# MiroBeno/Volume-Rendering

Hardware: AMD Instinct MI355X
Metric: Mrays/s (W*H / t_frame), 1024^3 volume @ 2048^2 viewport (higher is better)
Workload: dtype f32

## Files before the change

### include/vr_hip.h

```cpp
#ifndef VR_HIP_H
#define VR_HIP_H

#include <stddef.h>
#include <stdint.h>

#ifdef __cplusplus
extern "C" {
#endif

#define VR_TF_SIZE          128
#define VR_TF_RATIO         2
#define VR_ESL_VOLUME_DIMS  32
#define VR_ESL_VOLUME_SIZE  1024
#define VR_ESL_MIN_BLOCK    8

typedef enum vr_status {
	VR_OK               = 0,
	VR_ERR_INVALID      = 1,
	VR_ERR_NO_DEVICE    = 2,
	VR_ERR_ALLOC        = 3,
	VR_ERR_HIP          = 4,
	VR_ERR_NOT_READY    = 5
} vr_status;

// ... 72 lines not shown
int vr_hip_render_device(vr_ctx *ctx, const vr_params *params, void *dev_rgba, void *stream);

int vr_hip_render_mip(vr_ctx *ctx, const vr_params *params, uint8_t *host_rgba);
int vr_hip_render_mip_device(vr_ctx *ctx, const vr_params *params, void *dev_rgba, void *stream);

typedef struct vr_launch_info {
	uint32_t layout;
	uint32_t brick_plane;
	uint32_t lane_map;
	uint32_t phase_x, phase_y;
	uint32_t clamp_fetch;
	uint32_t tiles_x, tiles_y;
	uint32_t ordered;
	uint32_t straddle_permille;
	uint32_t column_voxels;
} vr_launch_info;
int vr_hip_last_launch(vr_ctx *ctx, vr_launch_info *out);

int vr_hip_timing(vr_ctx *ctx, vr_timing *out);
int vr_hip_timing_reset(vr_ctx *ctx);

int vr_hip_volume_minmax(vr_ctx *ctx, uint8_t *minmax_out, uint32_t *esl_block_dims_out, float *esl_block_size_out,
                         float *kernel_ms_out);
int vr_hip_volume_histogram(vr_ctx *ctx, uint64_t *hist256_out, float *kernel_ms_out);

int vr_hip_generate_volume(vr_ctx *ctx, uint32_t kind, uint32_t n, uint32_t seed, uint32_t bytes_per_voxel);
int vr_hip_download_volume(vr_ctx *ctx, void *host_out, uint64_t bytes);

typedef struct vr_multi vr_multi;
int  vr_hip_multi_create(int n, const int *devices, vr_multi **out);
// ... 62 lines not shown
```

### volume-rendering_amd/binding.py

```python
import ctypes as C
import os

SAMPLE_NEAREST = 0
SAMPLE_TRILINEAR = 1
SAMPLE_TRILINEAR_Q8 = 2
LAYOUT_LINEAR = 0
LAYOUT_BRICKED = 1
COPY_QUAD_XY, COPY_QUAD_XZ, COPY_QUAD_YZ, COPY_RUN_Z, COPY_RUN_Y, COPY_VOXEL, COPY_OCT, COPY_COL_X, COPY_COL_Y, COPY_COL_Z, COPY_ALL = 1, 2, 4, 8, 16, 32, 64, 128, 256, 512, 8191
COPY_COLV_X, COPY_COLV_Y, COPY_COLV_Z = 1024, 2048, 4096
COPY_NAMES = ("quad_xy", "quad_xz", "quad_yz", "run_z", "run_y", "voxel", "oct", "col_x", "col_y", "col_z", "colv_x", "colv_y", "colv_z")
COPY_KINDS = 13
TF_SIZE = 128
ESL_VOLUME_SIZE = 1024

_STATUS = {0: "VR_OK", 1: "VR_ERR_INVALID", 2: "VR_ERR_NO_DEVICE", 3: "VR_ERR_ALLOC", 4: "VR_ERR_HIP", 5: "VR_ERR_NOT_READY"}


class VrError(RuntimeError):
    def __init__(self, code, message=""):
        self.code = code
        super().__init__(f"{_STATUS.get(code, code)}: {message}" if message else _STATUS.get(code, str(code)))


class VrView(C.Structure):
# ... 22 lines not shown
class VrVolumeInfo(C.Structure):
    _fields_ = [("dim_x", C.c_uint32), ("dim_y", C.c_uint32), ("dim_z", C.c_uint32), ("bytes_per_voxel", C.c_uint32),
                ("layout", C.c_uint32), ("brick_copies", C.c_uint32), ("brick_copies_wanted", C.c_uint32), ("brick_planes", C.c_uint32),
                ("linear_resident", C.c_uint32), ("run_copy", C.c_uint32), ("linear_bytes", C.c_uint64), ("bricked_bytes", C.c_uint64),
                ("copies", C.c_uint32), ("copies_in_policy", C.c_uint32), ("copies_refused", C.c_uint32),
                ("build_ms", C.c_float * 13), ("upload_ms", C.c_float)]


class VrTiming(C.Structure):
    _fields_ = [("kernel_ms", C.c_float), ("total_ms", C.c_float), ("launches", C.c_uint64), ("kernel_ms_sum", C.c_double),
                ("kernel_ms_max", C.c_float), ("total_ms_max", C.c_float)]


class VrLaunchInfo(C.Structure):
    _fields_ = [(n, C.c_uint32) for n in ("layout", "brick_plane", "lane_map", "phase_x", "phase_y", "clamp_fetch", "tiles_x", "tiles_y",
                                          "ordered", "straddle_permille", "column_voxels")]


def library_path():
    return os.environ.get("VR_HIP_LIB") or os.path.join(os.path.dirname(os.path.abspath(__file__)), "libvr_hip.so")


_lib = None


def lib():
    global _lib
    if _lib is not None:
        return _lib
    import torch
    path = library_path()
# ... 84 lines not shown
```

### volume-rendering_amd/csrc/vr_device.h

```cpp
#pragma once

#include <hip/hip_runtime.h>
#include <stdint.h>
#include "../../include/vr_hip.h"

namespace vr {

constexpr uint32_t kMaxRaySteps = 1u << 22;

#ifndef VR_DEPTH
#define VR_DEPTH 5
#endif
constexpr int kDepth = VR_DEPTH, kSlots = kDepth + 1;
#ifndef VR_LAZY_EXIT
#define VR_LAZY_EXIT 1
#endif
#ifndef VR_RUN_DEPTH
#define VR_RUN_DEPTH VR_DEPTH
#endif
constexpr int kDepthTwoByte = 3;
constexpr int kRunDepth = VR_RUN_DEPTH, kMaxDepth = kRunDepth > kDepth ? kRunDepth : kDepth;
constexpr int kOverrunSteps = kMaxDepth + (VR_LAZY_EXIT ? kMaxDepth + 1 : 0);
constexpr int kLutPad = (kOverrunSteps * 5 + 2) / 3 + 2;
static_assert(kDepth >= 1 && kDepth <= 6 && kRunDepth >= 1 && kRunDepth <= 12, "prefetch depth");
// ... 26 lines not shown
	uint32_t dual_shift;
	uint32_t dual_bits[32];
	uint32_t col_axis;
	struct ColDenseSample {
		float ax, ay, az;
		float tf_scale;
		float max_x, max_y, max_z;
		float tf_zero_below;
		float light_kd, ray_threshold;
		uint32_t pad[2];
	} col_sample;
	struct ColDenseShade {
		float dir[3];  float kd_scaled;
		float light[3]; uint32_t nbu;
		float lh[3];   uint32_t nw;
		uint32_t dim[3], pad;
	} col_shade;
#ifdef VR_BOUNDS_CHECK
	uint64_t bc_base, bc_bytes;
	uint64_t bc_alt_bytes;
	uint32_t *bc_fault;
	uint32_t bc_ntiles;
#endif
};
#ifndef VR_TILE_ORDER
#define VR_TILE_ORDER 8
#endif
#ifndef VR_XCD_MODE
#define VR_XCD_MODE 5
#endif
inline void tile_number_to_xy(uint32_t tile, uint32_t tiles_x, uint32_t tiles_y, uint32_t *x, uint32_t *y) {
// ... 119 lines not shown
```

### volume-rendering_amd/csrc/vr_hip_api.cpp

```cpp
#include "vr_device.h"

#include <algorithm>
#include <chrono>
#include <cmath>
#include <cstdio>
#include <cstdlib>
#include <cstring>
#include <new>
#include <string>
#include <vector>

using namespace vr;

#ifndef VR_ORDER_ALWAYS
#define VR_ORDER_ALWAYS 0
#endif

namespace {

constexpr int kEventRing = 256;

struct EventPair { hipEvent_t start = nullptr, stop = nullptr; bool pending = false; };

}
// ... 349 lines not shown
}

#ifdef VR_BOUNDS_CHECK
hipError_t bounds_check_arm(vr_ctx *c, RayKernelArgs &a, const vr_params *p, const RaymarchPlan &plan, const void *brick_copy, uint32_t ntiles) {
	if (c->bc_fault == nullptr) {
		hipError_t e = hipMalloc((void **) &c->bc_fault, 8 * sizeof(uint32_t));
		if (e == hipSuccess) e = hipMemset(c->bc_fault, 0, 8 * sizeof(uint32_t));
		if (e != hipSuccess) return e;
	}
	const void *array = plan.reads_linear ? c->vol : brick_copy;
	const bool column = a.layout == kLayoutColumn || a.layout == kLayoutVoxCol;
	a.bc_base = (uint64_t) (uintptr_t) array - (column ? kColPadBytes : 0u);
	a.bc_bytes = plan.reads_linear ? (c->vol_elems + volume_tail_slack(c->dim[0], c->dim[1])) * c->bpv :
	             copy_bytes(c, copy_kind_of(a, p->sampling));
	if (column) a.bc_bytes += 2ull * kColPadBytes;
	a.bc_alt_bytes = a.alt_copy ? copy_bytes(c, kCopyRunY) : 0;
	a.bc_fault = c->bc_fault; a.bc_ntiles = ntiles;
	if (const char *e = getenv("VR_BC_SELFTEST")) if (atoi(e) == 1) a.bc_bytes /= 2;
	return hipSuccess;
}

int bounds_check_verdict(vr_ctx *c, hipStream_t stream, uint32_t layout) {
	uint32_t fault[6] = { 0, 0, 0, 0, 0, 0 };
	VR_TRY(c, hipStreamSynchronize(stream));
	VR_TRY(c, hipMemcpy(fault, c->bc_fault, sizeof fault, hipMemcpyDeviceToHost));
	if (fault[0] != 0u) {
		char msg[256];
		snprintf(msg, sizeof msg, "bounds check: code %u (1 table index [axis << 8], 2 offset, 3 address, 4 cost slot) workgroup %u thread %u value 0x%08x%08x limit %u, layout %u",
		         fault[0], fault[1], fault[2], fault[4], fault[3], fault[5], layout);
		(void) hipMemset(c->bc_fault, 0, 8 * sizeof(uint32_t));
		return fail(c, VR_ERR_HIP, msg);
// ... 90 lines not shown
		if (hit == nullptr) {
			const uint32_t straddle = choose_tile_mapping(a);
			hit = &c->map_cache[c->map_next];
			hit->straddle_permille = straddle;
			if (hit->dual_state != 0 || hit->order_tiles != 0) VR_TRY(c, drain(c));
			hit->dual_state = 0; hit->order_tiles = 0;
			constexpr uint32_t kMaps = sizeof c->map_cache / sizeof c->map_cache[0];
			c->map_next = (c->map_next + 1) % kMaps;
			if (c->map_cached < kMaps) c->map_cached++;
			hit->p = *p; memcpy(hit->dim, c->dim, sizeof c->dim);
			hit->lane_map = a.lane_map; hit->phase_x = a.phase_x; hit->phase_y = a.phase_y;
		}
		a.lane_map = hit->lane_map; a.phase_x = hit->phase_x; a.phase_y = hit->phase_y;
		if (run_if_unaligned && hit->straddle_permille > 150u && copy_possible(c, run_layout == kLayoutRunY ? kCopyRunY : kCopyRunZ)) a.layout = run_layout;
	}
	bool dual_analytic = false;
	int dual_stage = -1;
	const bool dual_test = c->brick_plane_force == (int) kPlanes + 4, dual_measured = c->brick_plane_force == (int) kPlanes + 3;
	if (dual_candidate && is_run_layout(a.layout) && !p->esl && p->ray_threshold >= 1.0f && !a.clamp_fetch && c->bpv == 1 &&
	    copy_possible(c, kCopyRunZ) && copy_possible(c, kCopyRunY)) {
		if (dual_test || dual_measured) {
			if (hit != nullptr && c->tile_scheduling == 1 && !VR_ORDER_ALWAYS) {
				dual_stage = dual_test ? 4 : (int) hit->dual_state;
				a.layout = dual_stage == 4 ? kLayoutRunDual : ((dual_stage & 1) ? kLayoutRunY : kLayoutRun);
			}
		} else {
			dual_analytic = true;
			a.layout = kLayoutRunDual;
		}
	}
	static const bool col_ert = [] { const char *e = getenv("VR_COL_ERT"); return e == nullptr || atoi(e) != 0; }();
	if (bricked && c->bpv == 1 && !c->force_wide && !p->view.perspective && !p->esl && (p->ray_threshold >= 1.0f || col_ert) &&
	    !a.clamp_fetch && c->column_force >= 0 && (c->brick_plane_force < 0 || c->column_force > 0)) {
		const float *d = va.d;
		const int m = va.major;
		const float advance = d[m] * p->ray_step;
		bool take = advance >= 1.0f / 64.0f && advance <= 1.0f && one_cell_per_pixel(p, half);
		if (c->column_force == 0)
			for (int i = 0; i < 3; i++) if (i != m && d[i] * 4.0f >= 0.45f) take = false;
		const bool nearest = p->sampling == VR_SAMPLE_NEAREST;
		bool voxcol = false;
		if (!nearest && c->column_copy == 0 && col_copy_bytes(c->dim, (uint32_t) m, true) < (1ull << 32)) {
			auto span = [&](int i) { return (int) std::floor(7.0f * (std::fabs(p->view.right_plane[i]) + std::fabs(p->view.up_plane[i])) * half[i]) + 4; };
			voxcol = span(m == 0 ? 1 : 0) * span(m == 2 ? 1 : 2) <= 64;
		}
		if (take && copy_possible(c, (nearest || voxcol ? kCopyColVoxX : kCopyColX) + (uint32_t) m)) {
			a.layout = voxcol ? kLayoutVoxCol : kLayoutColumn; a.col_axis = (uint32_t) m; a.brick_plane = (uint32_t) m;
			a.col_sample.ax = p->view.direction[0] * a.half_x; a.col_sample.ay = p->view.direction[1] * a.half_y; a.col_sample.az = p->view.direction[2] * a.half_z;
			a.col_sample.tf_scale = a.tf_scale; a.col_sample.tf_zero_below = a.tf_zero_below;
			a.col_sample.max_x = a.max_x; a.col_sample.max_y = a.max_y; a.col_sample.max_z = a.max_z;
			a.col_sample.light_kd = p->light_kd; a.col_sample.ray_threshold = p->ray_threshold;
			for (int i = 0; i < 3; i++) { a.col_shade.dir[i] = p->view.direction[i]; a.col_shade.light[i] = p->view.light_pos[i]; }
			a.col_shade.lh[0] = a.lh_x; a.col_shade.lh[1] = a.lh_y; a.col_shade.lh[2] = a.lh_z;
			a.col_shade.kd_scaled = a.kd_scaled;
			for (int i = 0; i < 3; i++) a.col_shade.dim[i] = c->dim[i];
			a.col_shade.nbu = col_blocks(c->dim[m == 0 ? 1 : 0]);
			a.col_shade.nw = col_windows(c->dim[m], nearest || voxcol ? kColVoxCells : kColCells);
			dual_analytic = false; dual_stage = -1;
		}
	}
	const void *brick_copy = nullptr;
	if (a.layout == kLayoutRunDual) {
		brick_copy = copy_for(c, kCopyRunZ);
		a.alt_copy = (uint64_t) (uintptr_t) copy_for(c, kCopyRunY);
		if (brick_copy == nullptr || a.alt_copy == 0) { a.layout = run_layout; dual_stage = -1; dual_analytic = false; brick_copy = nullptr; }
	}
	if (a.layout != kLayoutLinear && brick_copy == nullptr) {
		const uint32_t want = copy_kind_of(a, p->sampling);
		brick_copy = copy_for(c, want);
		if (brick_copy == nullptr && want != kCopyQuadXY) {
			a.layout = kLayoutBricked; a.brick_plane = kPlaneXY;
			forget_tile_mappings(c);
			brick_copy = copy_for(c, kCopyQuadXY);
		}
		if (brick_copy == nullptr) brick_copy = resident_fallback(c, p->sampling, true, a.layout);
	}
	if (c->tile_lane_map < 0 && is_run_layout(a.layout) && p->view.perspective && !p->esl) {
		if (va.along) {
			const int run_axis = a.layout == kLayoutRunY ? 1 : 2;
			const float across = std::fabs(p->view.right_plane[run_axis]), down = std::fabs(p->view.up_plane[run_axis]);
			a.lane_map = (a.lane_map & 3u) | ((down > across ? 2u : 1u) << 2);
		}
	}
	if (c->tile_lane_map < 0 && a.layout == kLayoutVoxel && p->view.perspective && (a.lane_map & 3u) == kLaneBlocks) {
		if (va.major != 2) a.lane_map = std::fabs(p->view.up_plane[2]) > std::fabs(p->view.right_plane[2]) ? kLaneColumns : kLaneRows;
	}
	const RaymarchPlan plan = plan_raymarch(a, brick_copy != nullptr, c->bpv);
	if (plan.reads_linear && c->vol == nullptr)
		return fail(c, VR_ERR_NOT_READY, "this frame needs the linear array, which was released (vr_hip_release_linear_copy): no resident brick copy "
		                                 "serves this sampling mode / addressing path — prepare it before releasing, or set the volume again");

// ... 110 lines not shown
	if (c->tile_scheduling == 2 && ntiles <= (1u << 20)) {
		if (c->cost_map_capacity < ntiles) {
			VR_TRY(c, drain(c));
			if (c->cost_map) (void) hipFree(c->cost_map);
			c->cost_map = nullptr; c->cost_map_capacity = 0;
			VR_TRY(c, hipMalloc((void **) &c->cost_map, (size_t) ntiles * 4));
			c->cost_map_capacity = ntiles;
		}
		VR_TRY(c, hipMemsetAsync(c->cost_map, 0, (size_t) ntiles * 4, stream));
		sched.cost = c->cost_map;
		c->cost_map_tiles_x = plan.tiles_x; c->cost_map_tiles_y = plan.tiles_y;
	}

	c->last_launch = vr_launch_info{ a.layout == kLayoutVoxCol ? (uint32_t) kLayoutColumn : a.layout, a.brick_plane, a.lane_map, a.phase_x, a.phase_y, a.clamp_fetch,
	                                 plan.tiles_x, plan.tiles_y, sched.order != nullptr ? 1u : 0u, hit != nullptr ? hit->straddle_permille : 1000u,
	                                 a.layout == kLayoutVoxCol ? 1u : 0u };

	uint64_t frame_seq = 0;
	const int rc = launch_timed(c, a, p, plan, brick_copy, stream, frame_seq, [&] { return launch_raymarch(a, c->vol, brick_copy, c->bpv, c->tf, c->esl, dev_rgba, sched, stream); });
	if (rc) return rc;
	if (dual_advance) {
		if (dual_stage == 3) VR_TRY(c, launch_tile_choice(hit->cost, hit->order + hit->capacity, hit->order, ntiles, stream));
		VR_TRY(c, hipEventRecord(hit->order_ready, stream));
		hit->order_stream = stream; hit->order_tiles = ntiles;
		hit->dual_state = (uint32_t) dual_stage + 1u;
	}
	if (read_slot != nullptr) read_slot->last_seq = frame_seq;
	if (record_slot != nullptr) {
		VR_TRY(c, launch_tile_order(record_slot->cost, record_slot->order, ntiles, stream));
		VR_TRY(c, hipEventRecord(record_slot->ready, stream));
		record_slot->valid = true; record_slot->ntiles = ntiles; record_slot->stream = stream; record_slot->issue_seq = record_slot->last_seq = frame_seq;
// ... 165 lines not shown
		if (hit == nullptr) {
			constexpr uint32_t kMaps = sizeof c->mip_map / sizeof c->mip_map[0];
			hit = &c->mip_map[c->mip_map_next];
			c->mip_map_next = (c->mip_map_next + 1) % kMaps;
			if (c->mip_mapped < kMaps) c->mip_mapped++;
			hit->straddle_permille = choose_tile_mapping(a);
			hit->p = *p; memcpy(hit->dim, c->dim, sizeof c->dim); hit->layout = a.layout; hit->brick_plane = a.brick_plane;
			hit->lane_map = a.lane_map; hit->phase_x = a.phase_x; hit->phase_y = a.phase_y;
		}
		a.lane_map = hit->lane_map; a.phase_x = hit->phase_x; a.phase_y = hit->phase_y; straddle = hit->straddle_permille;
	}
	const RaymarchPlan plan = plan_raymarch(a, brick_copy != nullptr, c->bpv);
	if (plan.reads_linear && c->vol == nullptr)
		return fail(c, VR_ERR_NOT_READY, "this MIP frame needs the linear array, which was released (vr_hip_release_linear_copy): no resident brick copy "
		                                 "serves this sampling mode / addressing path — prepare it before releasing, or set the volume again");
	c->last_launch = vr_launch_info{ plan.reads_linear ? (uint32_t) kLayoutLinear : a.layout, a.brick_plane, a.lane_map, a.phase_x, a.phase_y, 0u, plan.tiles_x, plan.tiles_y, 0u, straddle, 0u };
	uint64_t frame_seq = 0;
	return launch_timed(c, a, p, plan, brick_copy, stream, frame_seq, [&] { return launch_mip(a, c->vol, brick_copy, c->bpv, c->tf, a.p.esl ? c->mip_bounds : nullptr, dev_rgba, stream); });
}

int render_preamble(vr_ctx *c, const vr_params *p, const void *buffer, bool host_frame) {
	if (c == nullptr) return VR_ERR_INVALID;
	if (buffer == nullptr) return fail(c, VR_ERR_INVALID, "buffer is NULL");
	int rc = validate_params(c, p);
	if (rc) return rc;
	rc = ready(c);
	if (rc) return rc;
	if (host_frame && (c->fb == nullptr || (size_t) p->out_width * p->out_rows * 4 > c->fb_bytes))
		return fail(c, VR_ERR_NOT_READY, "output larger than the window buffer: call vr_hip_set_window first");
	VR_TRY(c, hipSetDevice(c->device));
	return VR_OK;
// ... 166 lines not shown
		return VR_OK;
	}
	c->column_force = 0;
	if (plane < -1 || plane > (int32_t) kPlanes + 4)
		return fail(c, VR_ERR_INVALID, "plane must be -1 (per view), 0 (x,y), 1 (x,z), 2 (y,z), 3 (run bricks along z), 4 (run bricks along y), 5 (oct bricks for every view of a "
		                               "2-byte volume), 6 (both run copies, chosen per tile by measurement, for every full-march view), 7 (both run copies on alternating tiles), "
		                               "8 (column windows for every orthogonal full-march frame) or 9 (never the column windows)");
	c->oct_always = plane == (int32_t) kPlanes + 2;
	c->brick_plane_force = c->oct_always ? -1 : plane;
	forget_tile_mappings(c);
	return VR_OK;
}

int vr_hip_set_column_copy(vr_ctx *c, uint32_t mode) {
	if (c == nullptr) return VR_ERR_INVALID;
	if (mode > 1u) return fail(c, VR_ERR_INVALID, "column copy must be 0 (voxel windows where a wave's columns fit, else quad-element windows) or 1 (quad-element windows)");
	c->column_copy = mode;
	return VR_OK;
}

int vr_hip_set_tile_scheduling(vr_ctx *c, uint32_t mode) {
	if (c == nullptr) return VR_ERR_INVALID;
	if (mode > 2u) return fail(c, VR_ERR_INVALID, "tile scheduling mode must be 0 (workgroup id), 1 (measured-cost order) or 2 (workgroup id + cost map)");
	c->tile_scheduling = mode;
	forget_recorded_orders(c);
	return VR_OK;
}

int vr_hip_last_launch(vr_ctx *c, vr_launch_info *out) {
	if (c == nullptr || out == nullptr) return VR_ERR_INVALID;
	*out = c->last_launch;
// ... 264 lines not shown
```

### volume-rendering_amd/csrc/vr_kernels.hip

```cpp
#include "vr_device.h"
#include <initializer_list>

namespace vr {

#define VR_FMA(a, b, c) __builtin_fmaf((a), (b), (c))

struct f3 { float x, y, z; };
struct f4 { float x, y, z, w; };

__device__ __forceinline__ f3 mk3(float x, float y, float z) { f3 r; r.x = x; r.y = y; r.z = z; return r; }
__device__ __forceinline__ f3 ld3(const float *p) { return mk3(p[0], p[1], p[2]); }
__device__ __forceinline__ float flmin(float a, float b) { return a < b ? a : b; }
__device__ __forceinline__ float flmax(float a, float b) { return a > b ? a : b; }

__device__ __forceinline__ uint32_t map_float_int(float f, uint32_t n) {
	int i = (int) (f * (float) n);
	if (i >= (int) n) i = (int) n - 1;
	if (i < 0) i = 0;
	return (uint32_t) i;
}

struct __attribute__((aligned(16))) LdsTables {
	f4 tf[VR_TF_SIZE + 1];
	f4 dtf[VR_TF_SIZE + 1];
// ... 997 lines not shown
	w.flips_u = __builtin_amdgcn_ballot_w64(w.cu0 != w.cu1); w.flips_v = __builtin_amdgcn_ballot_w64(w.cv0 != w.cv1);
	w.ok = w.ok && __builtin_amdgcn_ballot_w64((w.cu1 - w.cu0) * (w.cu1 - w.cu0) > 1 || (w.cv1 - w.cv0) * (w.cv1 - w.cv0) > 1) == 0ull;
}
__device__ __forceinline__ bool col_lane_offsets(const ColWave &w, uint64_t stride_u, uint64_t stride_v, int64_t &ref, int64_t &rel0) {
	ref = (int64_t) col_lateral_offset64((uint32_t) __builtin_amdgcn_readlane(w.cu0, w.leader), (uint32_t) __builtin_amdgcn_readlane(w.cv0, w.leader), stride_u, stride_v);
	rel0 = (int64_t) col_lateral_offset64((uint32_t) w.cu0, (uint32_t) w.cv0, stride_u, stride_v) - ref;
	const int64_t du64 = (int64_t) col_axis_offset64((uint32_t) w.cu1, stride_u, kColWindowBytes) - (int64_t) col_axis_offset64((uint32_t) w.cu0, stride_u, kColWindowBytes);
	const int64_t dv64 = (int64_t) col_axis_offset64((uint32_t) w.cv1, stride_v, kColRowBytes) - (int64_t) col_axis_offset64((uint32_t) w.cv0, stride_v, kColRowBytes);
	const int64_t lim = 1ll << 28;
	return __builtin_amdgcn_ballot_w64(rel0 <= -lim || rel0 >= lim || du64 <= -lim || du64 >= lim || dv64 <= -lim || dv64 >= lim) == 0ull;
}
__device__ __forceinline__ uint64_t col_scalar_base(const uint8_t *copy, int64_t ref) {
	const uint64_t b = (uint64_t) (uintptr_t) copy + (uint64_t) ref - (1ull << 30);
	return ((uint64_t) rfl((uint32_t) (b >> 32)) << 32) | rfl((uint32_t) b);
}

struct ColBatch {
	float kvec, knext;
	int wvec;
	template <class W> __device__ __forceinline__ void refill(float step, uint32_t lane_i, W cell_to_window) {
		const float kbase = knext;
		const float k1 = kbase + step, delta = k1 - kbase, low = step - delta;
		const uint32_t e = __float_as_uint(kbase) >> 23;
		const float half_ulp = __uint_as_float((e > 24u ? e - 24u : 1u) << 23);
		const float kend = VR_FMA(64.0f, delta, kbase);
		const bool fast = rfl((e > 24u && (__float_as_uint(kend) >> 23) == e && __builtin_fabsf(low) != half_ulp && delta > 0.0f) ? 1u : 0u) != 0u;
		if (fast) {
			kvec = VR_FMA((float) lane_i, delta, kbase);
			knext = uni(kend);
		} else {
// ... 105 lines not shown
#if defined(VR_BOUNDS_CHECK)
		managed_load128(dst, VR_BC_ADDRESS(a, s_base + lane_offset, 16u));
#else
		managed_load128_s(dst, lane_offset, s_base);
#endif
		woff += dsign * (int) kColBlockBytes;
	}
	__device__ __forceinline__ bool careful(const ColEvents &e) {
		if (!FLIPS) return false;
		const int key = issue_key - (DEPTH + 1);
		while (key > cons_event) { cons_at++; cons_event = __builtin_amdgcn_readlane(e.events, cons_at & 63); }
		return key == cons_event;
	}
};

template <int SAMPLING, int M, class ShadeCorners>
__device__ __forceinline__ void col_tri_sample(const RayKernelArgs &a, uint32_t w0, uint32_t w1, float k, const f3 &B, ColRay &ray, uint64_t &live, f4 &acc,
                                               const f4 (&tf_l)[VR_TF_SIZE + 1], const f4 (&dtf_l)[VR_TF_SIZE + 1], const f4 (&org_l)[512], ShadeCorners shade_corners) {
	constexpr bool kQ8 = SAMPLING == VR_SAMPLE_TRILINEAR_Q8;
	if ((__builtin_amdgcn_uicmp((w0 | w1) & a.skip_mask, a.skip_cmp, kIcmpNE) & live) != 0ull && VR_OPEN_LANES(acc.w, live) != 0ull) {
		ColConstArgs q = col_dense_args();
		RayKernelArgs::ColDenseSample ds;
		ds.ax = q->col_sample.ax; ds.ay = q->col_sample.ay; ds.az = q->col_sample.az; ds.tf_scale = q->col_sample.tf_scale;
		ds.max_x = q->col_sample.max_x; ds.max_y = q->col_sample.max_y; ds.max_z = q->col_sample.max_z; ds.tf_zero_below = q->col_sample.tf_zero_below;
		ds.light_kd = q->col_sample.light_kd; ds.ray_threshold = q->col_sample.ray_threshold;
		hold_scalars(ds.ax, ds.ay, ds.az, ds.tf_scale, ds.max_x, ds.max_y, ds.max_z, ds.tf_zero_below, ds.light_kd, ds.ray_threshold);
		live &= __builtin_amdgcn_fcmpf(k, ray.ky, kFcmpOLE);
		const float xb = VR_FMA(k, ds.ax, B.x), yb = VR_FMA(k, ds.ay, B.y), zb = VR_FMA(k, ds.az, B.z);
		const float raw = col_resolve<M, kQ8>(w0, w1, ds.max_x, ds.max_y, ds.max_z, xb, yb, zb);
		const float tb = __builtin_amdgcn_fmed3f(VR_FMA(raw, ds.tf_scale, -0.5f), 0.0f, (float) (VR_TF_SIZE - 1));
		if ((__builtin_amdgcn_fcmpf(tb, ds.tf_zero_below, kFcmpOGE) & live) != 0ull) {
			f4 c;
			{
				const uint32_t i = (uint32_t) (int) tb;
				const float w = filter_weight<kQ8>(__builtin_amdgcn_fractf(tb));
				const f4 c0 = tf_l[i], dc = dtf_l[i];
				c.x = VR_FMA(w, dc.x, c0.x); c.y = VR_FMA(w, dc.y, c0.y); c.z = VR_FMA(w, dc.z, c0.z); c.w = VR_FMA(w, dc.w, c0.w);
			}
			const uint64_t shaded = ds.light_kd > 0.01f ? (__builtin_amdgcn_fcmpf(c.w, 0.05f, kFcmpOGT) & live) : 0ull;
			if (shaded != 0ull) {
				const f3 org = col_origin_again(org_l, ray.org_slot);
				RayKernelArgs::ColDenseShade dh;
				for (int i = 0; i < 3; i++) { dh.dir[i] = q->col_shade.dir[i]; dh.light[i] = q->col_shade.light[i]; dh.lh[i] = q->col_shade.lh[i]; }
				dh.kd_scaled = q->col_shade.kd_scaled; dh.nbu = q->col_shade.nbu; dh.nw = q->col_shade.nw;
				const uint8_t *const copy_p = ((ColConstKernelArguments) q)->copy;
				hold_scalars(dh.dir[0], dh.dir[1], dh.dir[2], dh.kd_scaled, dh.light[0], dh.light[1], dh.light[2], dh.lh[0], dh.lh[1], dh.lh[2]);
				hold_scalars(dh.nbu, dh.nw, (uint64_t) (uintptr_t) copy_p);
				const f3 p3 = march_point<SAMPLING>(org, mk3(dh.dir[0], dh.dir[1], dh.dir[2]), k);
				const f3 d = mk3(dh.light[0] - p3.x, dh.light[1] - p3.y, dh.light[2] - p3.z);
				const float inv = rsqrt_nr(VR_FMA(d.z, d.z, VR_FMA(d.y, d.y, d.x * d.x)));
				const float sx = VR_FMA(d.x * inv, dh.lh[0], xb), sy = VR_FMA(d.y * inv, dh.lh[1], yb), sz = VR_FMA(d.z * inv, dh.lh[2], zb);
				uint32_t l0, l1;
				shade_corners(copy_p, ds, dh, sx, sy, sz, l0, l1);
				const float raw_l = col_resolve<M, kQ8>(l0, l1, ds.max_x, ds.max_y, ds.max_z, sx, sy, sz);
				const float diffuse = select_lanes(shaded, (raw_l - raw) * dh.kd_scaled);
				c.x += diffuse; c.y += diffuse; c.z += diffuse;
			}
			const float t = select_lanes(live, 1 - acc.w);
			acc.x = VR_FMA(c.x, t, acc.x); acc.y = VR_FMA(c.y, t, acc.y); acc.z = VR_FMA(c.z, t, acc.z); acc.w = VR_FMA(c.w, t, acc.w);
			live &= ~__builtin_amdgcn_fcmpf(acc.w, ds.ray_threshold, kFcmpOGT);
// ... 30 lines not shown
	if (ray.alive_mask == 0ull) { if (ray.in_frame) out[ray.out_index] = 0u; return; }

	const f3 A = mk3(uni(ray.dir.x * a.half_x), uni(ray.dir.y * a.half_y), uni(ray.dir.z * a.half_z));
	const f3 B = mk3(VR_FMA(ray.origin.x, a.half_x, a.off_x), VR_FMA(ray.origin.y, a.half_y, a.off_y), VR_FMA(ray.origin.z, a.half_z, a.off_z));
	const float Am = comp3<M>(A), Au = comp3<U>(A), Av = comp3<V>(A);
	const float Bm = comp3<M>(B), Bu = comp3<U>(B), Bv = comp3<V>(B);
	const uint32_t dim_u = U == 0 ? a.dim_x : a.dim_y, dim_m = M == 0 ? a.dim_x : (M == 1 ? a.dim_y : a.dim_z);
	const float max_u = U == 0 ? a.max_x : a.max_y, max_v = V == 1 ? a.max_y : a.max_z;
	const uint32_t nbu = col_blocks(dim_u), nw = col_windows(dim_m);
	const uint64_t stride_u = (uint64_t) nw * kColBlockBytes, stride_v = (uint64_t) nbu * stride_u;

	f4 acc; acc.x = acc.y = acc.z = acc.w = 0.0f;
	uint64_t live = ray.alive_mask;
	float k = ray.kx;

	auto pair_address = [&](const uint8_t *copy_p, float mx, float my, float mz, uint32_t blocks_u, uint32_t windows, float xb, float yb, float zb) {
		const int ix = (int) __builtin_amdgcn_fmed3f(xb, 0.0f, mx), iy = (int) __builtin_amdgcn_fmed3f(yb, 0.0f, my), iz = (int) __builtin_amdgcn_fmed3f(zb, 0.0f, mz);
		const uint32_t iu = (uint32_t) (U == 0 ? ix : iy), iv = (uint32_t) (V == 1 ? iy : iz), im = (uint32_t) (M == 0 ? ix : (M == 1 ? iy : iz));
		const uint32_t wq = __umulhi(im, 0xAAAAAAABu) >> 1, sub = im - wq * 3u;
		const uint32_t block = col_lateral_block(iu, iv, blocks_u) * windows + wq;
		const uint32_t in_block = col_in_block(iu, iv) + sub * 4u;
		const uint8_t *p = copy_p + ((uint64_t) block * kColBlockBytes + in_block);
		return VR_BC_POINTER(a, const uint8_t *, p, 8u);
	};
	auto coords = [&](ColConstArgs q, float kk, float &xb, float &yb, float &zb) {
		xb = VR_FMA(kk, q->col_sample.ax, B.x); yb = VR_FMA(kk, q->col_sample.ay, B.y); zb = VR_FMA(kk, q->col_sample.az, B.z);
	};
	auto fetch_at = [&](float kk, uint32_t &w0, uint32_t &w1) {
		ColConstArgs q = col_dense_args();
		float xb, yb, zb;
		coords(q, kk, xb, yb, zb);
		const uint2 both = *(const uint2 *) pair_address(((ColConstKernelArguments) q)->copy, q->col_sample.max_x, q->col_sample.max_y, q->col_sample.max_z, q->col_shade.nbu, q->col_shade.nw, xb, yb, zb);
		w0 = both.x; w1 = both.y;
	};
	auto fetch_at_managed = [&](float kk, uint64_t &both) {
		ColConstArgs q = col_dense_args();
		float xb, yb, zb;
		coords(q, kk, xb, yb, zb);
		managed_load64(both, (uint64_t) (uintptr_t) pair_address(((ColConstKernelArguments) q)->copy, q->col_sample.max_x, q->col_sample.max_y, q->col_sample.max_z, q->col_shade.nbu, q->col_shade.nw, xb, yb, zb));
	};
	auto sample = [&](uint32_t w0, uint32_t w1) {
		col_tri_sample<SAMPLING, M>(a, w0, w1, k, B, ray, live, acc, tf_l, dtf_l, org_l,
			[&](const uint8_t *copy_p, const RayKernelArgs::ColDenseSample &ds, const RayKernelArgs::ColDenseShade &dh, float sx, float sy, float sz, uint32_t &l0, uint32_t &l1) {
				const uint2 both = *(const uint2 *) pair_address(copy_p, ds.max_x, ds.max_y, ds.max_z, dh.nbu, dh.nw, sx, sy, sz);
				l0 = both.x; l1 = both.y;
			});
	};

	auto cell = [&](float kk, float Ac, float Bc, float maxc) { return (int) __builtin_amdgcn_fmed3f(VR_FMA(kk, Ac, Bc), 0.0f, maxc); };
	auto cell_u = [&](float kk) { return cell(kk, Au, Bu, max_u); };
	auto cell_v = [&](float kk) { return cell(kk, Av, Bv, max_v); };
	ColWave wv;
	col_wave_eligibility(ray, Bm, __builtin_fabsf(Am) * ray.step, cell_u, cell_v, wv);
	int64_t ref, rel0;
	const bool ok = col_lane_offsets(wv, stride_u, stride_v, ref, rel0) && wv.ok;
	const float Bm_l = wv.cm_l;

	const bool has_flips = (wv.flips_u | wv.flips_v) != 0ull;
	auto per_lane_march = [&]() {
// ... 236 lines not shown
			col_drain(slot);
		}
	} else per_lane_march();
	col_store(ray, acc);
}

#ifndef VR_VOXCOL_DEPTH
#define VR_VOXCOL_DEPTH 3
#endif
#ifndef VR_VOXCOL_WAVES
#define VR_VOXCOL_WAVES VR_COL_WAVES
#endif
constexpr int kVoxColDepth = VR_VOXCOL_DEPTH, kVoxColSlots = kVoxColDepth + 1;
static_assert(kVoxColDepth >= 2 && 2 * kVoxColSlots + kVoxColDepth + 4 <= 64, "kColPadBytes");

template <int SAMPLING, int M, bool FLIPS>
__global__ __launch_bounds__(512) __attribute__((amdgpu_waves_per_eu(VR_VOXCOL_WAVES, 8)))
void voxcol_tri_kernel(const RayKernelArgs a, const uint8_t *__restrict__ copy, const float *__restrict__ tf_g, uint32_t *__restrict__ out) {
	constexpr int U = M == 0 ? 1 : 0, V = M == 2 ? 1 : 2;
	constexpr int kCells = (int) kColVoxCells;
	__shared__ f4 tf_l[VR_TF_SIZE + 1], dtf_l[VR_TF_SIZE + 1];
	__shared__ f4 org_l[512];
	stage_tf_with_deltas(tf_l, dtf_l, tf_g);
	__syncthreads();
	ColRay ray;
	col_ray_setup(a, org_l, ray);
	if (ray.alive_mask == 0ull) { if (ray.in_frame) out[ray.out_index] = 0u; return; }

	const f3 A = mk3(uni(ray.dir.x * a.half_x), uni(ray.dir.y * a.half_y), uni(ray.dir.z * a.half_z));
	const f3 B = mk3(VR_FMA(ray.origin.x, a.half_x, a.off_x), VR_FMA(ray.origin.y, a.half_y, a.off_y), VR_FMA(ray.origin.z, a.half_z, a.off_z));
	const float Am = comp3<M>(A), Au = comp3<U>(A), Av = comp3<V>(A);
	const float Bm = comp3<M>(B), Bu = comp3<U>(B), Bv = comp3<V>(B);
	const uint32_t dim_u = U == 0 ? a.dim_x : a.dim_y, dim_v = V == 1 ? a.dim_y : a.dim_z, dim_m = M == 0 ? a.dim_x : (M == 1 ? a.dim_y : a.dim_z);
	const float max_u = U == 0 ? a.max_x : a.max_y, max_v = V == 1 ? a.max_y : a.max_z;
	const uint32_t nbu = col_blocks(dim_u), nw = col_windows(dim_m, kColVoxCells);
	const uint64_t stride_u = (uint64_t) nw * kColBlockBytes, stride_v = (uint64_t) nbu * stride_u;

	f4 acc; acc.x = acc.y = acc.z = acc.w = 0.0f;
	uint64_t live = ray.alive_mask;
	float k = ray.kx;

	auto corners_at = [&](const uint8_t *copy_p, float mx, float my, float mz, uint32_t blocks_u, uint32_t windows, float xb, float yb, float zb,
	                      uint32_t &w0, uint32_t &w1) {
		const uint32_t ix = (uint32_t) (int) __builtin_amdgcn_fmed3f(xb, 0.0f, mx), iy = (uint32_t) (int) __builtin_amdgcn_fmed3f(yb, 0.0f, my),
		               iz = (uint32_t) (int) __builtin_amdgcn_fmed3f(zb, 0.0f, mz);
		const float fu = U == 0 ? mx : my, fv = V == 1 ? my : mz, fm = M == 0 ? mx : (M == 1 ? my : mz);
		const uint32_t iu = U == 0 ? ix : iy, iv = V == 1 ? iy : iz, im = M == 0 ? ix : (M == 1 ? iy : iz);
		const uint32_t iu1 = iu + ((float) iu < fu ? 1u : 0u), iv1 = iv + ((float) iv < fv ? 1u : 0u), im1 = im + ((float) im < fm ? 1u : 0u);
		auto along = [](uint32_t m) { return (m >> 4) * kColBlockBytes + (m & 15u); };
		auto ld = [&](uint32_t off) { return (uint32_t) *VR_BC_POINTER(a, const uint8_t *, copy_p + off, 1u); };
		const uint32_t l00 = col_lateral_offset(iu, iv, blocks_u, windows), l10 = col_lateral_offset(iu1, iv, blocks_u, windows),
		               l01 = col_lateral_offset(iu, iv1, blocks_u, windows), l11 = col_lateral_offset(iu1, iv1, blocks_u, windows), m0 = along(im), m1 = along(im1);
		w0 = ld(l00 + m0) | (ld(l10 + m0) << 8) | (ld(l01 + m0) << 16) | (ld(l11 + m0) << 24);
		w1 = ld(l00 + m1) | (ld(l10 + m1) << 8) | (ld(l01 + m1) << 16) | (ld(l11 + m1) << 24);
	};
	auto fetch_at = [&](float kk, uint32_t &w0, uint32_t &w1) {
		ColConstArgs q = col_dense_args();
		const float xb = VR_FMA(kk, q->col_sample.ax, B.x), yb = VR_FMA(kk, q->col_sample.ay, B.y), zb = VR_FMA(kk, q->col_sample.az, B.z);
		corners_at(((ColConstKernelArguments) q)->copy, q->col_sample.max_x, q->col_sample.max_y, q->col_sample.max_z, q->col_shade.nbu, q->col_shade.nw, xb, yb, zb, w0, w1);
	};
	auto sample = [&](uint32_t w0, uint32_t w1) {
		col_tri_sample<SAMPLING, M>(a, w0, w1, k, B, ray, live, acc, tf_l, dtf_l, org_l,
			[&](const uint8_t *copy_p, const RayKernelArgs::ColDenseSample &ds, const RayKernelArgs::ColDenseShade &dh, float sx, float sy, float sz, uint32_t &l0, uint32_t &l1) {
				corners_at(copy_p, ds.max_x, ds.max_y, ds.max_z, dh.nbu, dh.nw, sx, sy, sz, l0, l1);
			});
	};

	auto cell = [&](float kk, float Ac, float Bc, float maxc) { return (int) __builtin_amdgcn_fmed3f(VR_FMA(kk, Ac, Bc), 0.0f, maxc); };
	auto cell_u = [&](float kk) { return cell(kk, Au, Bu, max_u); };
	auto cell_v = [&](float kk) { return cell(kk, Av, Bv, max_v); };
	ColWave wv;
	col_wave_eligibility(ray, Bm, __builtin_fabsf(Am) * ray.step, cell_u, cell_v, wv);
	const float Bm_l = wv.cm_l;
	const int cu0 = wv.cu0, cu1 = wv.cu1, cv0 = wv.cv0, cv1 = wv.cv1;
	const uint64_t flips = wv.flips_u | wv.flips_v;
	bool ok = wv.ok && (FLIPS || flips == 0ull);
	int ru0 = cu0 < cu1 ? cu0 : cu1, ru1 = (cu0 > cu1 ? cu0 : cu1) + 1, rv0 = cv0 < cv1 ? cv0 : cv1, rv1 = (cv0 > cv1 ? cv0 : cv1) + 1;
// ... 90 lines not shown
					const uint32_t p01 = (uint32_t) __builtin_amdgcn_ds_bpermute((int) (at + rw4), pair), p11 = (uint32_t) __builtin_amdgcn_ds_bpermute((int) (at + rw4 + 4u), pair);
					const uint32_t t0 = __builtin_amdgcn_perm(p10, p00, 0x05010400u), t1 = __builtin_amdgcn_perm(p11, p01, 0x05010400u);
					sample(__builtin_amdgcn_perm(t1, t0, 0x05040100u), __builtin_amdgcn_perm(t1, t0, 0x07060302u));
				});
			}
			carry = o.x;
			cur += dsign;
		};
		while (live != 0ull && guard > 0) {
			static_for<0, kVoxColSlots>(window_step);
			guard -= kVoxColSlots;
		}
		col_drain(slot, carry);
	} else per_lane_march();
	col_store(ray, acc);
}

#ifndef VR_MIP_BATCH
#define VR_MIP_BATCH 4
#endif
constexpr int kMipBatch = VR_MIP_BATCH;
extern __shared__ __attribute__((aligned(16))) uint8_t mip_bound_lds[];

template <int SAMPLING, int BPV, int ADDR, int LAYOUT>
__global__ __launch_bounds__(LutCfg<(LAYOUT != kLayoutLinear ? ADDR : kAddrWide)>::threads)
void mip_kernel(const RayKernelArgs a, const void *__restrict__ vol, const float *__restrict__ tf_g, const uint8_t *__restrict__ bounds_g,
                uint32_t *__restrict__ out) {
	typedef LutCfg<(LAYOUT != kLayoutLinear ? ADDR : kAddrWide)> L;
	constexpr uint32_t kThreads = L::threads;
	constexpr bool kNearest = SAMPLING == VR_SAMPLE_NEAREST, kQ8 = SAMPLING == VR_SAMPLE_TRILINEAR_Q8;
// ... 260 lines not shown
		plan.tile_h = threads / 32u;
		return plan;
	});
}

hipError_t launch_raymarch(const RayKernelArgs &args, const void *linear, const void *bricked, uint32_t bpv, const float *tf,
                           const uint32_t *esl, void *out, TileSchedule sched, hipStream_t stream) {
	if (bricked != nullptr && (args.layout == kLayoutColumn || args.layout == kLayoutVoxCol)) {
		RayKernelArgs a = args;
		tile_grid(a.p.out_width, a.p.out_rows, a.phase_x, a.phase_y, 512u, a.tiles_x, a.tiles_y);
		const dim3 grid(a.tiles_x * a.tiles_y), block(512);
		auto go = [&](auto kernel) { hipLaunchKernelGGL(kernel, grid, block, 0, stream, a, (const uint8_t *) bricked, tf, (uint32_t *) out); };
		const uint32_t m = a.col_axis;
		const bool flips = a.p.view.direction[m == 0u ? 1 : 0] != 0.0f || a.p.view.direction[m == 2u ? 1 : 2] != 0.0f;
		const bool voxels = a.layout == kLayoutVoxCol;
		dispatch_axis_flag(m, flips, [&](auto axis, auto flag) {
			constexpr int AX = decltype(axis)::value;
			constexpr bool FL = decltype(flag)::value;
			constexpr int T = VR_SAMPLE_TRILINEAR, Q8 = VR_SAMPLE_TRILINEAR_Q8;
			if (a.p.sampling == VR_SAMPLE_NEAREST) go(colmarch_nearest_kernel<AX, FL>);
			else if (a.p.sampling == VR_SAMPLE_TRILINEAR_Q8) { if (voxels) go(voxcol_tri_kernel<Q8, AX, FL>); else go(colmarch_kernel<Q8, AX, FL>); }
			else if (voxels) go(voxcol_tri_kernel<T, AX, FL>); else go(colmarch_kernel<T, AX, FL>);
		});
		return hipGetLastError();
	}
	return select_variant(args, bricked != nullptr, bpv, [&](auto sampling, auto voxel, auto addr, auto layout, bool reads_linear) {
		constexpr int SAMPLING = decltype(sampling)::value, BPV = decltype(voxel)::value, ADDR = decltype(addr)::value, LAYOUT = decltype(layout)::value;
		constexpr uint32_t threads = variant_threads<ADDR, LAYOUT>();
		RayKernelArgs a = args;
		tile_grid(a.p.out_width, a.p.out_rows, a.phase_x, a.phase_y, threads, a.tiles_x, a.tiles_y);
#ifndef VR_RUN_LDS_PAD
#define VR_RUN_LDS_PAD 16384
#endif
#ifndef VR_PAD_LAYOUTS
#define VR_PAD_LAYOUTS ((1u << kLayoutRun) | (1u << kLayoutRunY) | (1u << kLayoutRunDual))
#endif
		const uint32_t dynamic_lds = ((VR_PAD_LAYOUTS >> LAYOUT) & 1u) && !a.p.esl ? VR_RUN_LDS_PAD : 0;
// ... 579 lines not shown
```

Baseline: 2134.

## Read lit voxel-column frames from quad-element column copy for shading gradients

When the voxel-column layout is chosen for a lit frame (light_kd above a threshold, default column_copy mode), the kernel now reads corner data from the quad-element column copy (alt_copy) using 8-byte pair loads, instead of per-voxel window addressing. A new kernel variant and a windows count (nwq) are added, and dispatch selects it when alt_copy is set. This trades the voxel-window copy's cheaper addressing for the quad copy's fewer, wider loads during gradient shading. It also requires the quad column copy to be resident alongside the voxel copy, and the bounds-check size now follows it.

```diff
diff --git a/include/vr_hip.h b/include/vr_hip.h
--- a/include/vr_hip.h
+++ b/include/vr_hip.h
@@ -110,6 +110,7 @@
 	uint32_t ordered;
 	uint32_t straddle_permille;
 	uint32_t column_voxels;
+	uint32_t column_shade_pairs;
 } vr_launch_info;
 int vr_hip_last_launch(vr_ctx *ctx, vr_launch_info *out);
 
diff --git a/volume-rendering_amd/binding.py b/volume-rendering_amd/binding.py
--- a/volume-rendering_amd/binding.py
+++ b/volume-rendering_amd/binding.py
@@ -60,7 +60,7 @@
 
 class VrLaunchInfo(C.Structure):
     _fields_ = [(n, C.c_uint32) for n in ("layout", "brick_plane", "lane_map", "phase_x", "phase_y", "clamp_fetch", "tiles_x", "tiles_y",
-                                          "ordered", "straddle_permille", "column_voxels")]
+                                          "ordered", "straddle_permille", "column_voxels", "column_shade_pairs")]
 
 
 def library_path():
diff --git a/volume-rendering_amd/csrc/vr_device.h b/volume-rendering_amd/csrc/vr_device.h
--- a/volume-rendering_amd/csrc/vr_device.h
+++ b/volume-rendering_amd/csrc/vr_device.h
@@ -64,7 +64,7 @@
 		float dir[3];  float kd_scaled;
 		float light[3]; uint32_t nbu;
 		float lh[3];   uint32_t nw;
-		uint32_t dim[3], pad;
+		uint32_t dim[3], nwq;
 	} col_shade;
 #ifdef VR_BOUNDS_CHECK
 	uint64_t bc_base, bc_bytes;
diff --git a/volume-rendering_amd/csrc/vr_hip_api.cpp b/volume-rendering_amd/csrc/vr_hip_api.cpp
--- a/volume-rendering_amd/csrc/vr_hip_api.cpp
+++ b/volume-rendering_amd/csrc/vr_hip_api.cpp
@@ -387,7 +387,7 @@
 	a.bc_bytes = plan.reads_linear ? (c->vol_elems + volume_tail_slack(c->dim[0], c->dim[1])) * c->bpv :
 	             copy_bytes(c, copy_kind_of(a, p->sampling));
 	if (column) a.bc_bytes += 2ull * kColPadBytes;
-	a.bc_alt_bytes = a.alt_copy ? copy_bytes(c, kCopyRunY) : 0;
+	a.bc_alt_bytes = a.alt_copy ? copy_bytes(c, a.layout == kLayoutVoxCol ? kCopyColX + a.col_axis : (uint32_t) kCopyRunY) : 0;
 	a.bc_fault = c->bc_fault; a.bc_ntiles = ntiles;
 	if (const char *e = getenv("VR_BC_SELFTEST")) if (atoi(e) == 1) a.bc_bytes /= 2;
 	return hipSuccess;
@@ -508,7 +508,7 @@
 		a.lane_map = hit->lane_map; a.phase_x = hit->phase_x; a.phase_y = hit->phase_y;
 		if (run_if_unaligned && hit->straddle_permille > 150u && copy_possible(c, run_layout == kLayoutRunY ? kCopyRunY : kCopyRunZ)) a.layout = run_layout;
 	}
-	bool dual_analytic = false;
+	bool dual_analytic = false, shade_pairs = false;
 	int dual_stage = -1;
 	const bool dual_test = c->brick_plane_force == (int) kPlanes + 4, dual_measured = c->brick_plane_force == (int) kPlanes + 3;
 	if (dual_candidate && is_run_layout(a.layout) && !p->esl && p->ray_threshold >= 1.0f && !a.clamp_fetch && c->bpv == 1 &&
@@ -534,7 +534,7 @@
 			for (int i = 0; i < 3; i++) if (i != m && d[i] * 4.0f >= 0.45f) take = false;
 		const bool nearest = p->sampling == VR_SAMPLE_NEAREST;
 		bool voxcol = false;
-		if (!nearest && c->column_copy == 0 && col_copy_bytes(c->dim, (uint32_t) m, true) < (1ull << 32)) {
+		if (!nearest && c->column_copy != 1u && col_copy_bytes(c->dim, (uint32_t) m, true) < (1ull << 32)) {
 			auto span = [&](int i) { return (int) std::floor(7.0f * (std::fabs(p->view.right_plane[i]) + std::fabs(p->view.up_plane[i])) * half[i]) + 4; };
 			voxcol = span(m == 0 ? 1 : 0) * span(m == 2 ? 1 : 2) <= 64;
 		}
@@ -550,6 +550,8 @@
 			for (int i = 0; i < 3; i++) a.col_shade.dim[i] = c->dim[i];
 			a.col_shade.nbu = col_blocks(c->dim[m == 0 ? 1 : 0]);
 			a.col_shade.nw = col_windows(c->dim[m], nearest || voxcol ? kColVoxCells : kColCells);
+			a.col_shade.nwq = col_windows(c->dim[m]);
+			shade_pairs = voxcol && p->light_kd > 0.01f && c->column_copy == 0;
 			dual_analytic = false; dual_stage = -1;
 		}
 	}
@@ -569,6 +571,7 @@
 		}
 		if (brick_copy == nullptr) brick_copy = resident_fallback(c, p->sampling, true, a.layout);
 	}
+	if (shade_pairs && a.layout == kLayoutVoxCol && brick_copy != nullptr) a.alt_copy = (uint64_t) (uintptr_t) copy_for(c, kCopyColX + a.col_axis);
 	if (c->tile_lane_map < 0 && is_run_layout(a.layout) && p->view.perspective && !p->esl) {
 		if (va.along) {
 			const int run_axis = a.layout == kLayoutRunY ? 1 : 2;
@@ -709,7 +712,7 @@
 
 	c->last_launch = vr_launch_info{ a.layout == kLayoutVoxCol ? (uint32_t) kLayoutColumn : a.layout, a.brick_plane, a.lane_map, a.phase_x, a.phase_y, a.clamp_fetch,
 	                                 plan.tiles_x, plan.tiles_y, sched.order != nullptr ? 1u : 0u, hit != nullptr ? hit->straddle_permille : 1000u,
-	                                 a.layout == kLayoutVoxCol ? 1u : 0u };
+	                                 a.layout == kLayoutVoxCol ? 1u : 0u, a.layout == kLayoutVoxCol && a.alt_copy != 0 ? 1u : 0u };
 
 	uint64_t frame_seq = 0;
 	const int rc = launch_timed(c, a, p, plan, brick_copy, stream, frame_seq, [&] { return launch_raymarch(a, c->vol, brick_copy, c->bpv, c->tf, c->esl, dev_rgba, sched, stream); });
@@ -905,7 +908,7 @@
 	if (plan.reads_linear && c->vol == nullptr)
 		return fail(c, VR_ERR_NOT_READY, "this MIP frame needs the linear array, which was released (vr_hip_release_linear_copy): no resident brick copy "
 		                                 "serves this sampling mode / addressing path — prepare it before releasing, or set the volume again");
-	c->last_launch = vr_launch_info{ plan.reads_linear ? (uint32_t) kLayoutLinear : a.layout, a.brick_plane, a.lane_map, a.phase_x, a.phase_y, 0u, plan.tiles_x, plan.tiles_y, 0u, straddle, 0u };
+	c->last_launch = vr_launch_info{ plan.reads_linear ? (uint32_t) kLayoutLinear : a.layout, a.brick_plane, a.lane_map, a.phase_x, a.phase_y, 0u, plan.tiles_x, plan.tiles_y, 0u, straddle, 0u, 0u };
 	uint64_t frame_seq = 0;
 	return launch_timed(c, a, p, plan, brick_copy, stream, frame_seq, [&] { return launch_mip(a, c->vol, brick_copy, c->bpv, c->tf, a.p.esl ? c->mip_bounds : nullptr, dev_rgba, stream); });
 }
@@ -1102,7 +1105,8 @@
 
 int vr_hip_set_column_copy(vr_ctx *c, uint32_t mode) {
 	if (c == nullptr) return VR_ERR_INVALID;
-	if (mode > 1u) return fail(c, VR_ERR_INVALID, "column copy must be 0 (voxel windows where a wave's columns fit, else quad-element windows) or 1 (quad-element windows)");
+	if (mode > 2u) return fail(c, VR_ERR_INVALID, "column copy must be 0 (voxel windows where a wave's columns fit, else quad-element windows; lit frames shade from the "
+	                                              "quad-element windows), 1 (quad-element windows) or 2 (as 0, shading from the voxel windows)");
 	c->column_copy = mode;
 	return VR_OK;
 }
diff --git a/volume-rendering_amd/csrc/vr_kernels.hip b/volume-rendering_amd/csrc/vr_kernels.hip
--- a/volume-rendering_amd/csrc/vr_kernels.hip
+++ b/volume-rendering_amd/csrc/vr_kernels.hip
@@ -1035,6 +1035,18 @@
 	const uint64_t b = (uint64_t) (uintptr_t) copy + (uint64_t) ref - (1ull << 30);
 	return ((uint64_t) rfl((uint32_t) (b >> 32)) << 32) | rfl((uint32_t) b);
 }
+template <int M>
+__device__ __forceinline__ const uint8_t *col_pair_address(const RayKernelArgs &a, const uint8_t *copy_p, float mx, float my, float mz, uint32_t blocks_u, uint32_t windows,
+                                                           float xb, float yb, float zb) {
+	constexpr int U = M == 0 ? 1 : 0, V = M == 2 ? 1 : 2;
+	const int ix = (int) __builtin_amdgcn_fmed3f(xb, 0.0f, mx), iy = (int) __builtin_amdgcn_fmed3f(yb, 0.0f, my), iz = (int) __builtin_amdgcn_fmed3f(zb, 0.0f, mz);
+	const uint32_t iu = (uint32_t) (U == 0 ? ix : iy), iv = (uint32_t) (V == 1 ? iy : iz), im = (uint32_t) (M == 0 ? ix : (M == 1 ? iy : iz));
+	const uint32_t wq = __umulhi(im, 0xAAAAAAABu) >> 1, sub = im - wq * 3u;
+	const uint32_t block = col_lateral_block(iu, iv, blocks_u) * windows + wq;
+	const uint32_t in_block = col_in_block(iu, iv) + sub * 4u;
+	const uint8_t *p = copy_p + ((uint64_t) block * kColBlockBytes + in_block);
+	return VR_BC_POINTER(a, const uint8_t *, p, 8u);
+}
 
 struct ColBatch {
 	float kvec, knext;
@@ -1170,7 +1182,7 @@
 	}
 };
 
-template <int SAMPLING, int M, class ShadeCorners>
+template <int SAMPLING, int M, bool PAIR_COPY = false, class ShadeCorners>
 __device__ __forceinline__ void col_tri_sample(const RayKernelArgs &a, uint32_t w0, uint32_t w1, float k, const f3 &B, ColRay &ray, uint64_t &live, f4 &acc,
                                                const f4 (&tf_l)[VR_TF_SIZE + 1], const f4 (&dtf_l)[VR_TF_SIZE + 1], const f4 (&org_l)[512], ShadeCorners shade_corners) {
 	constexpr bool kQ8 = SAMPLING == VR_SAMPLE_TRILINEAR_Q8;
@@ -1198,8 +1210,8 @@
 				const f3 org = col_origin_again(org_l, ray.org_slot);
 				RayKernelArgs::ColDenseShade dh;
 				for (int i = 0; i < 3; i++) { dh.dir[i] = q->col_shade.dir[i]; dh.light[i] = q->col_shade.light[i]; dh.lh[i] = q->col_shade.lh[i]; }
-				dh.kd_scaled = q->col_shade.kd_scaled; dh.nbu = q->col_shade.nbu; dh.nw = q->col_shade.nw;
-				const uint8_t *const copy_p = ((ColConstKernelArguments) q)->copy;
+				dh.kd_scaled = q->col_shade.kd_scaled; dh.nbu = q->col_shade.nbu; dh.nw = PAIR_COPY ? q->col_shade.nwq : q->col_shade.nw;
+				const uint8_t *const copy_p = PAIR_COPY ? (const uint8_t *) (uintptr_t) q->alt_copy : ((ColConstKernelArguments) q)->copy;
 				hold_scalars(dh.dir[0], dh.dir[1], dh.dir[2], dh.kd_scaled, dh.light[0], dh.light[1], dh.light[2], dh.lh[0], dh.lh[1], dh.lh[2]);
 				hold_scalars(dh.nbu, dh.nw, (uint64_t) (uintptr_t) copy_p);
 				const f3 p3 = march_point<SAMPLING>(org, mk3(dh.dir[0], dh.dir[1], dh.dir[2]), k);
@@ -1260,15 +1272,6 @@
 	uint64_t live = ray.alive_mask;
 	float k = ray.kx;
 
-	auto pair_address = [&](const uint8_t *copy_p, float mx, float my, float mz, uint32_t blocks_u, uint32_t windows, float xb, float yb, float zb) {
-		const int ix = (int) __builtin_amdgcn_fmed3f(xb, 0.0f, mx), iy = (int) __builtin_amdgcn_fmed3f(yb, 0.0f, my), iz = (int) __builtin_amdgcn_fmed3f(zb, 0.0f, mz);
-		const uint32_t iu = (uint32_t) (U == 0 ? ix : iy), iv = (uint32_t) (V == 1 ? iy : iz), im = (uint32_t) (M == 0 ? ix : (M == 1 ? iy : iz));
-		const uint32_t wq = __umulhi(im, 0xAAAAAAABu) >> 1, sub = im - wq * 3u;
-		const uint32_t block = col_lateral_block(iu, iv, blocks_u) * windows + wq;
-		const uint32_t in_block = col_in_block(iu, iv) + sub * 4u;
-		const uint8_t *p = copy_p + ((uint64_t) block * kColBlockBytes + in_block);
-		return VR_BC_POINTER(a, const uint8_t *, p, 8u);
-	};
 	auto coords = [&](ColConstArgs q, float kk, float &xb, float &yb, float &zb) {
 		xb = VR_FMA(kk, q->col_sample.ax, B.x); yb = VR_FMA(kk, q->col_sample.ay, B.y); zb = VR_FMA(kk, q->col_sample.az, B.z);
 	};
@@ -1276,19 +1279,19 @@
 		ColConstArgs q = col_dense_args();
 		float xb, yb, zb;
 		coords(q, kk, xb, yb, zb);
-		const uint2 both = *(const uint2 *) pair_address(((ColConstKernelArguments) q)->copy, q->col_sample.max_x, q->col_sample.max_y, q->col_sample.max_z, q->col_shade.nbu, q->col_shade.nw, xb, yb, zb);
+		const uint2 both = *(const uint2 *) col_pair_address<M>(a, ((ColConstKernelArguments) q)->copy, q->col_sample.max_x, q->col_sample.max_y, q->col_sample.max_z, q->col_shade.nbu, q->col_shade.nw, xb, yb, zb);
 		w0 = both.x; w1 = both.y;
 	};
 	auto fetch_at_managed = [&](float kk, uint64_t &both) {
 		ColConstArgs q = col_dense_args();
 		float xb, yb, zb;
 		coords(q, kk, xb, yb, zb);
-		managed_load64(both, (uint64_t) (uintptr_t) pair_address(((ColConstKernelArguments) q)->copy, q->col_sample.max_x, q->col_sample.max_y, q->col_sample.max_z, q->col_shade.nbu, q->col_shade.nw, xb, yb, zb));
+		managed_load64(both, (uint64_t) (uintptr_t) col_pair_address<M>(a, ((ColConstKernelArguments) q)->copy, q->col_sample.max_x, q->col_sample.max_y, q->col_sample.max_z, q->col_shade.nbu, q->col_shade.nw, xb, yb, zb));
 	};
 	auto sample = [&](uint32_t w0, uint32_t w1) {
 		col_tri_sample<SAMPLING, M>(a, w0, w1, k, B, ray, live, acc, tf_l, dtf_l, org_l,
 			[&](const uint8_t *copy_p, const RayKernelArgs::ColDenseSample &ds, const RayKernelArgs::ColDenseShade &dh, float sx, float sy, float sz, uint32_t &l0, uint32_t &l1) {
-				const uint2 both = *(const uint2 *) pair_address(copy_p, ds.max_x, ds.max_y, ds.max_z, dh.nbu, dh.nw, sx, sy, sz);
+				const uint2 both = *(const uint2 *) col_pair_address<M>(a, copy_p, ds.max_x, ds.max_y, ds.max_z, dh.nbu, dh.nw, sx, sy, sz);
 				l0 = both.x; l1 = both.y;
 			});
 	};
@@ -1555,13 +1558,11 @@
 constexpr int kVoxColDepth = VR_VOXCOL_DEPTH, kVoxColSlots = kVoxColDepth + 1;
 static_assert(kVoxColDepth >= 2 && 2 * kVoxColSlots + kVoxColDepth + 4 <= 64, "kColPadBytes");
 
-template <int SAMPLING, int M, bool FLIPS>
-__global__ __launch_bounds__(512) __attribute__((amdgpu_waves_per_eu(VR_VOXCOL_WAVES, 8)))
-void voxcol_tri_kernel(const RayKernelArgs a, const uint8_t *__restrict__ copy, const float *__restrict__ tf_g, uint32_t *__restrict__ out) {
+template <int SAMPLING, int M, bool FLIPS, bool PAIRS>
+__device__ __forceinline__ void voxcol_march(const RayKernelArgs &a, const uint8_t *__restrict__ copy, const float *__restrict__ tf_g, uint32_t *__restrict__ out,
+                                             f4 (&tf_l)[VR_TF_SIZE + 1], f4 (&dtf_l)[VR_TF_SIZE + 1], f4 (&org_l)[512]) {
 	constexpr int U = M == 0 ? 1 : 0, V = M == 2 ? 1 : 2;
 	constexpr int kCells = (int) kColVoxCells;
-	__shared__ f4 tf_l[VR_TF_SIZE + 1], dtf_l[VR_TF_SIZE + 1];
-	__shared__ f4 org_l[512];
 	stage_tf_with_deltas(tf_l, dtf_l, tf_g);
 	__syncthreads();
 	ColRay ray;
@@ -1583,6 +1584,11 @@
 
 	auto corners_at = [&](const uint8_t *copy_p, float mx, float my, float mz, uint32_t blocks_u, uint32_t windows, float xb, float yb, float zb,
 	                      uint32_t &w0, uint32_t &w1) {
+		if constexpr (PAIRS) {
+			const uint2 both = *(const uint2 *) col_pair_address<M>(a, copy_p, mx, my, mz, blocks_u, windows, xb, yb, zb);
+			w0 = both.x; w1 = both.y;
+			return;
+		}
 		const uint32_t ix = (uint32_t) (int) __builtin_amdgcn_fmed3f(xb, 0.0f, mx), iy = (uint32_t) (int) __builtin_amdgcn_fmed3f(yb, 0.0f, my),
 		               iz = (uint32_t) (int) __builtin_amdgcn_fmed3f(zb, 0.0f, mz);
 		const float fu = U == 0 ? mx : my, fv = V == 1 ? my : mz, fm = M == 0 ? mx : (M == 1 ? my : mz);
@@ -1598,10 +1604,11 @@
 	auto fetch_at = [&](float kk, uint32_t &w0, uint32_t &w1) {
 		ColConstArgs q = col_dense_args();
 		const float xb = VR_FMA(kk, q->col_sample.ax, B.x), yb = VR_FMA(kk, q->col_sample.ay, B.y), zb = VR_FMA(kk, q->col_sample.az, B.z);
-		corners_at(((ColConstKernelArguments) q)->copy, q->col_sample.max_x, q->col_sample.max_y, q->col_sample.max_z, q->col_shade.nbu, q->col_shade.nw, xb, yb, zb, w0, w1);
+		corners_at(PAIRS ? (const uint8_t *) (uintptr_t) q->alt_copy : ((ColConstKernelArguments) q)->copy, q->col_sample.max_x, q->col_sample.max_y, q->col_sample.max_z,
+		           q->col_shade.nbu, PAIRS ? q->col_shade.nwq : q->col_shade.nw, xb, yb, zb, w0, w1);
 	};
 	auto sample = [&](uint32_t w0, uint32_t w1) {
-		col_tri_sample<SAMPLING, M>(a, w0, w1, k, B, ray, live, acc, tf_l, dtf_l, org_l,
+		col_tri_sample<SAMPLING, M, PAIRS>(a, w0, w1, k, B, ray, live, acc, tf_l, dtf_l, org_l,
 			[&](const uint8_t *copy_p, const RayKernelArgs::ColDenseSample &ds, const RayKernelArgs::ColDenseShade &dh, float sx, float sy, float sz, uint32_t &l0, uint32_t &l1) {
 				corners_at(copy_p, ds.max_x, ds.max_y, ds.max_z, dh.nbu, dh.nw, sx, sy, sz, l0, l1);
 			});
@@ -1722,6 +1729,21 @@
 		col_drain(slot, carry);
 	} else per_lane_march();
 	col_store(ray, acc);
+}
+
+template <int SAMPLING, int M, bool FLIPS>
+__global__ __launch_bounds__(512) __attribute__((amdgpu_waves_per_eu(VR_VOXCOL_WAVES, 8)))
+void voxcol_tri_kernel(const RayKernelArgs a, const uint8_t *__restrict__ copy, const float *__restrict__ tf_g, uint32_t *__restrict__ out) {
+	__shared__ f4 tf_l[VR_TF_SIZE + 1], dtf_l[VR_TF_SIZE + 1];
+	__shared__ f4 org_l[512];
+	voxcol_march<SAMPLING, M, FLIPS, false>(a, copy, tf_g, out, tf_l, dtf_l, org_l);
+}
+template <int SAMPLING, int M, bool FLIPS>
+__global__ __launch_bounds__(512) __attribute__((amdgpu_waves_per_eu(VR_VOXCOL_WAVES, 8)))
+void voxcol_pairs_kernel(const RayKernelArgs a, const uint8_t *__restrict__ copy, const float *__restrict__ tf_g, uint32_t *__restrict__ out) {
+	__shared__ f4 tf_l[VR_TF_SIZE + 1], dtf_l[VR_TF_SIZE + 1];
+	__shared__ f4 org_l[512];
+	voxcol_march<SAMPLING, M, FLIPS, true>(a, copy, tf_g, out, tf_l, dtf_l, org_l);
 }
 
 #ifndef VR_MIP_BATCH
@@ -2012,13 +2034,14 @@
 		const uint32_t m = a.col_axis;
 		const bool flips = a.p.view.direction[m == 0u ? 1 : 0] != 0.0f || a.p.view.direction[m == 2u ? 1 : 2] != 0.0f;
 		const bool voxels = a.layout == kLayoutVoxCol;
+		const bool pairs = voxels && a.alt_copy != 0ull;
 		dispatch_axis_flag(m, flips, [&](auto axis, auto flag) {
 			constexpr int AX = decltype(axis)::value;
 			constexpr bool FL = decltype(flag)::value;
 			constexpr int T = VR_SAMPLE_TRILINEAR, Q8 = VR_SAMPLE_TRILINEAR_Q8;
 			if (a.p.sampling == VR_SAMPLE_NEAREST) go(colmarch_nearest_kernel<AX, FL>);
-			else if (a.p.sampling == VR_SAMPLE_TRILINEAR_Q8) { if (voxels) go(voxcol_tri_kernel<Q8, AX, FL>); else go(colmarch_kernel<Q8, AX, FL>); }
-			else if (voxels) go(voxcol_tri_kernel<T, AX, FL>); else go(colmarch_kernel<T, AX, FL>);
+			else if (a.p.sampling == VR_SAMPLE_TRILINEAR_Q8) { if (pairs) go(voxcol_pairs_kernel<Q8, AX, FL>); else if (voxels) go(voxcol_tri_kernel<Q8, AX, FL>); else go(colmarch_kernel<Q8, AX, FL>); }
+			else if (pairs) go(voxcol_pairs_kernel<T, AX, FL>); else if (voxels) go(voxcol_tri_kernel<T, AX, FL>); else go(colmarch_kernel<T, AX, FL>);
 		});
 		return hipGetLastError();
 	}
```

New measurement: 2236, median of 6. 1.05x the previous value.
